# featureform/embeddinghub

Measured on NVIDIA H100. Metric: k-NN queries/s, higher is better.
Workload: dtype f32

## Files before the change

embeddinghub_b200/csrc/api.cu:

```cuda
#include "index_impl.h"

namespace ehb {
thread_local std::string g_err;
int fail(int code, const std::string& msg) {
  g_err = msg;
  return code;
}
const std::string& last_error_text() { return g_err; }
}
using ehb::fail;

ehb_index::~ehb_index() {
  slots.clear();
  if (bf_ev0) cudaEventDestroy(bf_ev0);
  if (bf_ev1) cudaEventDestroy(bf_ev1);
  if (stream) cudaStreamDestroy(stream);
}

ehb::GraphView ehb_index::view() const {
  ehb::GraphView g;
  g.vecs = vecs.p;
  g.links0 = links0.p;
  g.up_off = up_off.p;
  g.links_up = links_up.p;
// ... 24 lines not shown
  const uint64_t need = std::max<uint64_t>(cap, 1) * (dpad + sizeof(float4)) + (256ull << 20);
  bool ok = cudaMemGetInfo(&fr, &tot) == cudaSuccess && fr >= need;
  if (ok) {
    cudaError_t e = x_i8.grow(std::max<uint64_t>(cap, 1) * dpad, 0, -1, stream);
    if (e == cudaSuccess) e = x_i8t.grow(std::max<uint64_t>(cap, 1), 0, -1, stream);
    if (e == cudaSuccess) e = ehb::launch_to_i8(vecs.p, dpad, x_i8.p, x_i8t.p, n, stream);
    if (e == cudaSuccess) e = cudaStreamSynchronize(stream);
    screen_copy = e == cudaSuccess;
    if (!screen_copy) {
      x_i8.release();
      x_i8t.release();
      ok = false;
    }
  }
  if (!ok) {
    (void)cudaGetLastError();
    ehb::g_err.clear();
    screen_no_room = true;
  }
  return EHB_OK;
}

ehb::WalkCfg ehb_index::walk_cfg(uint32_t ef_eff, uint32_t smem_list, uint64_t jobs, uint32_t team, bool bf16,
                                 bool dense) const {
  ehb::WalkCfg c;
  const uint32_t vbytes = dpad * (bf16 ? 2u : 4u);
  c.lcap = smem_list;
  c.staged = ehb::row_lpv(vbytes) == 32 ? 1 : 0;
  c.dcap = n_deleted ? ehb::kDeletedQueue : 0;
  c.prefetch = o_walk_prefetch ? 1 : 0;
  c.dense = dense ? 1 : 0;
  const uint32_t warp_target = c.dense ? 20u : 16u;
  uint32_t nslots = std::max(4u, std::min(32u, 24576u / vbytes));
  uint32_t ng = 2;
  uint32_t g = std::max(4u, nslots / ng / 4 * 4);
  if (t_slots) g = std::min(32u, t_slots);
  if (t_groups) ng = std::min(8u, t_groups);
  c.G = std::max(1u, g);
  c.NG = std::max(1u, ng);
  const uint32_t roomy = 2u * M0 * ef_eff + 64u, tight = std::max(256u, M0 * ef_eff / 4u);
  uint32_t hs = roomy;
  if (t_hash_bits) {
    hs = 1u << t_hash_bits;
  } else {
    uint64_t ctas = (jobs + team - 1) / std::max(team, 1u);
    uint32_t want = (uint32_t)std::min<uint64_t>((ctas + sms - 1) / sms, c.staged ? 5u : warp_target / team);
    want = std::max(want, 4u);
    c.hash_size = 0;
    uint32_t fixed = ehb::warp_smem_bytes(c, vbytes) * team + 1024u + (smem_list ? 256u : 0u);
    uint32_t per_cta = (227u * 1024u) / want;
    uint32_t avail = per_cta > fixed + 1024u ? (per_cta - fixed) / 4u : 256u;
    hs = std::min(roomy, std::max(tight, avail));
    if (n_deleted) hs = roomy;
  }
  c.hash_size = ehb::align_up(std::max(hs, 256u), 32);
  while (ehb::warp_smem_bytes(c, vbytes) + 256 > 200 * 1024 && c.hash_size > 512)
    c.hash_size = ehb::align_up(c.hash_size / 2, 32);
  return c;
}

uint32_t ehb_index::wpb_for(const ehb::WalkCfg& c, uint32_t extra, bool bf16) const {
  uint32_t w = t_wpb ? t_wpb : 1;
  const uint32_t vbytes = dpad * (bf16 ? 2u : 4u);
  while (w > 1 && (size_t)(ehb::warp_smem_bytes(c, vbytes) + extra) * w > 220 * 1024) w >>= 1;
  return w;
}

constexpr uint64_t kTeamWideMaxQueries = 132u * 3u;

ehb::WalkPlan ehb_index::walk_plan(uint64_t nq, uint32_t ef_eff, bool bf16) const {
  ehb::WalkPlan p;
  p.bf16 = bf16;
  const uint32_t row_bytes = dpad * (bf16 ? 2u : 4u);
  p.lpv = ehb::row_lpv(row_bytes);
  p.nq = ehb::row_nq(dpad, row_bytes);
  p.kpl = ehb::kpl_for(ef_eff);
  p.hasdel = n_deleted != 0;
  uint32_t team = t_team;
  if (team == 0) team = nq <= (uint64_t)sms * 3 ? 4 : (nq <= (uint64_t)sms * 7 ? 2 : 1);
  if (dpad > 256 || ef_eff > 256 || n_deleted) team = 1;
  if (bf16) team = 1;
  p.T = team;
  const bool wide = team == 2 || (team == 4 && nq <= kTeamWideMaxQueries);
  p.U = team == 1 ? 0 : (uint32_t)ehb::eval_u(p.nq, wide ? 1 : 2);
  if (team > 1)
    p.form = ehb::WalkForm::team;
  else if (nq >= 20ull * (uint64_t)sms && ehb::dense_form(bf16, p.lpv, p.nq, p.kpl, p.hasdel))
    p.form = ehb::WalkForm::dense;
  else
    p.form = ehb::WalkForm::plain;
  p.screen = !bf16 && team == 1 && screen_copy && walk_screens(nq);
  p.cfg = walk_cfg(ef_eff, 0, nq * team, team, bf16, p.form == ehb::WalkForm::dense);
  p.wpb = wpb_for(p.cfg, 0, bf16);
  return p;
}

int ehb_index::ensure_capacity(uint64_t want) {
  if (want <= cap) return EHB_OK;
  uint64_t nc = std::max<uint64_t>(cap ? cap : 1, 1);
  while (nc < want) nc *= 2;
  if (nc >= 0x7FFFFFFFull) return fail(EHB_ERR_INVALID, "capacity must stay below 2^31 vectors per index");
  CU(vecs.grow(nc * dpad, n * dpad, -1, stream));
  CU(labels.grow(nc, n, -1, stream));
  CU(levels.grow(nc, n, 0, stream));
  CU(deleted.grow(nc, n, 0, stream));
  CU(links0.grow(nc * M0, n * M0, 0xFF, stream));
  CU(up_off.grow(nc, n, 0xFF, stream));
  if (shadow) {
    CU(x_bf16.grow(nc * dpad, n * dpad, -1, stream));
    CU(x_norm.grow(nc, n, -1, stream));
  }
  if (screen_copy) {
    CU(x_i8.grow(nc * dpad, n * dpad, -1, stream));
    CU(x_i8t.grow(nc, n, -1, stream));
  }
// ... 1128 lines not shown
```

embeddinghub_b200/csrc/index_impl.h:

```cpp
#pragma once
#include <cuda_runtime.h>

#include <algorithm>
#include <atomic>
#include <cmath>
#include <condition_variable>
#include <cstdio>
#include <cstdlib>
#include <cstring>
#include <deque>
#include <memory>
#include <mutex>
#include <new>
#include <random>
#include <shared_mutex>
#include <string>
#include <unordered_map>
#include <vector>

#include "../../include/ehb200.h"
#include "kernels.h"

namespace ehb {

// ... 214 lines not shown
  bool shadow = false;
  ehb::DevBuf<int8_t> x_i8;
  ehb::DevBuf<float4> x_i8t;
  bool screen_copy = false;

  ehb::DevBuf<uint32_t> b_edge_row, b_edge_src, b_row_cnt, b_row_fill, b_row_start, b_touched, b_seg_src, b_counters,
      b_ids, b_upd_cand;
  ehb::DevBuf<float> b_edge_dist, b_seg_dist, b_stage_in;

  uint32_t t_slots = 0, t_groups = 0, t_hash_bits = 0, t_wpb = 0, t_team = 0;
  uint32_t o_build_frac = 0;
  bool o_bf16_unfused = false;
  bool o_combine = true;
  bool o_walk_prefetch = false;
  int o_walk_screen = -1;
  bool screen_no_room = false;

  std::default_random_engine level_rng;

  ~ehb_index();

  ehb::GraphView view() const;
  ehb::WalkCfg walk_cfg(uint32_t ef_eff, uint32_t smem_list, uint64_t jobs, uint32_t team, bool bf16 = false,
                        bool dense = false) const;
  uint32_t wpb_for(const ehb::WalkCfg& c, uint32_t extra, bool bf16 = false) const;
  ehb::WalkPlan walk_plan(uint64_t nq, uint32_t ef_eff, bool bf16) const;
  int ensure_capacity(uint64_t want);
  int ensure_upper(uint64_t want_rows);
  int draw_level();
  bool find_id(uint64_t label, uint32_t* id) const;
  int add_rows(uint64_t cnt, const float* src, bool src_is_device, const uint64_t* lab);
  int remove_labels(uint64_t cnt, const uint64_t* lab);
  int ensure_build_scratch(uint64_t edges, uint32_t batch, bool updates);
  ehb::BuildBuffers build_buffers(uint64_t edges);
  ehb::BuildGraph build_graph() const;
  int build();
  int compact();
  bool needs_build() const { return n_linked != n || !pending_updates.empty(); }
  int ensure_built(std::shared_lock<ehb::RwLock>& lk, bool bf16 = false, bool screen = false);
  bool walk_screens(uint64_t nq) const;
  int try_screen_copy();
  int ensure_shadow(std::shared_lock<ehb::RwLock>& lk);
  int create_shadow();
  int derive_rows(uint64_t first, uint64_t cnt);
  void drop_derived();
  int acquire_slot(ehb::SearchSlot** out);
  void release_slot(ehb::SearchSlot* sl, cudaStream_t used);
// ... 8 lines not shown
```

embeddinghub_b200/csrc/search_impl.cuh:

```cuda
#pragma once
#include "kernels.h"

namespace ehb {

template <int LPV, int NQ, int KPL, bool HASDEL, int UDIV, class RowT>
__device__ __forceinline__ void search_body(const GraphView& g, const WalkCfg& cfg, const float* __restrict__ queries,
                                            uint32_t nq, uint32_t k, uint32_t ef, const ResultSink& sink,
                                            uint32_t* __restrict__ out_counts, uint32_t* __restrict__ stats,
                                            uint32_t warp_smem) {
  extern __shared__ __align__(128) unsigned char smem[];
  const uint32_t w = threadIdx.x >> 5;
  const uint32_t q = blockIdx.x * (blockDim.x >> 5) + w;
  if (q >= nq) return;
  constexpr bool kKeys = !std::is_same<RowT, float>::value;
  WarpCtx c;
  ctx_init(c, smem + (size_t)w * warp_smem, cfg, g.dpad, (uint32_t)sizeof(RowT));
  float4 qr[NQ];
  load_query_regs<LPV, NQ, RowT>(qr, queries + (size_t)q * g.dim, g.dim, c.lane);
  WalkCounters wc = {0, 0, 0, 0};
  UList<KPL> ul;
  ul_clear<KPL>(ul, ef, c.lane);
  if (g.n != 0) {
    uint32_t cur = g.entry;
    if (c.lane == 0) c.cand_id[0] = cur;
    __syncwarp();
    eval_candidates<LPV, NQ, UDIV>(c, walk_rows<RowT>(g), qr, 1, g.metric);
    float curdist = c.cand_dist[0];
    __syncwarp();
    wc.evals = 1;
    greedy_descent<LPV, NQ, UDIV, RowT>(c, g, qr, cur, curdist, g.max_level, 0, wc);
    beam_search<LPV, NQ, KPL, true, HASDEL, UDIV, RowT>(c, g, qr, ul, cur, curdist, 0, ef, kInvalid, wc);
  }
  uint64_t rk[KPL];
#pragma unroll
  for (int s = 0; s < KPL; ++s) rk[s] = kMaxKey;
  uint32_t found = 0;
  for (uint32_t i = 0; i < k; ++i) {
    uint64_t key = ul_extract_min<KPL>(ul, c.lane);
    if (key == kMaxKey) break;
#pragma unroll
    for (int s = 0; s < KPL; ++s)
      if ((i >> 5) == (uint32_t)s && (i & 31u) == c.lane) rk[s] = key;
    found++;
  }
  if constexpr (kKeys) {
#pragma unroll
    for (int s = 0; s < KPL; ++s) {
      const uint32_t idx = (uint32_t)s * 32u + c.lane;
      if ((uint32_t)s * 32u < k && idx < k) sink.keys[(size_t)q * k + idx] = rk[s];
    }
  } else {
#pragma unroll
    for (int s = 0; s < KPL; ++s) {
      const uint32_t idx = (uint32_t)s * 32u + c.lane;
// ... 11 lines not shown
    if (sink.qs) {
      __threadfence_system();
      __syncwarp();
      if (c.lane == 0) {
        const uint32_t slice = q / sink.qs;
        const uint32_t size = min(sink.qs, nq - slice * sink.qs);
        if (atomicAdd(&sink.slice_count[slice], 1u) + 1u == size) {
          sink.slice_count[slice] = 0;
          __threadfence_system();
          for (uint32_t t = 1; t < sink.n; ++t) st_release_sys(sink.flags[t] + slice, sink.epoch);
        }
      }
    }
  }
  if (c.lane == 0) {
    if (out_counts) out_counts[q] = found;
    if (stats) {
      ((uint4*)stats)[2 * q] = make_uint4(wc.hops_upper, wc.hops_base, wc.evals, wc.overflow);
      ((uint4*)stats)[2 * q + 1] = make_uint4(wc.screened, wc.survivors, 0u, 0u);
    }
  }
}

template <class RowT, int LPV, int NQ>
constexpr int kWalkMinBlocks = std::is_same<RowT, float>::value && !screen_shape(LPV, NQ) ? 0 : 1;
template <int LPV, int NQ, int KPL, bool HASDEL, class RowT>
__global__ void __launch_bounds__(128, (kWalkMinBlocks<RowT, LPV, NQ>))
    hnsw_search_kernel(GraphView g, WalkCfg cfg, const float* __restrict__ queries, uint32_t nq, uint32_t k, uint32_t ef,
                       const __grid_constant__ ResultSink sink, uint32_t* __restrict__ out_counts,
                       uint32_t* __restrict__ stats, uint32_t warp_smem) {
  search_body<LPV, NQ, KPL, HASDEL, 1, RowT>(g, cfg, queries, nq, k, ef, sink, out_counts, stats, warp_smem);
}

template <int LPV, int NQ, int KPL, class RowT>
__global__ void __launch_bounds__(128, 5) hnsw_search_dense_kernel(GraphView g, WalkCfg cfg,
                                                                   const float* __restrict__ queries, uint32_t nq,
                                                                   uint32_t k, uint32_t ef,
                                                                   const __grid_constant__ ResultSink sink,
                                                                   uint32_t* __restrict__ out_counts,
                                                                   uint32_t* __restrict__ stats, uint32_t warp_smem) {
  search_body<LPV, NQ, KPL, false, 2, RowT>(g, cfg, queries, nq, k, ef, sink, out_counts, stats, warp_smem);
}

template <int LPV, int NQ, int KPL, class RowT>
cudaError_t launch_search_t(const WalkPlan& p, const GraphView& g, const float* queries, uint32_t nq, uint32_t k,
                            uint32_t ef, const ResultSink& sink, uint32_t* out_counts, uint32_t* stats,
                            cudaStream_t s) {
  constexpr bool kBf16 = !std::is_same<RowT, float>::value;
  const uint32_t wpb = p.wpb;
  uint32_t wsm = warp_smem_bytes(p.cfg, g.dpad * (uint32_t)sizeof(RowT));
  size_t smem = (size_t)wsm * wpb;
  dim3 grid((nq + wpb - 1) / wpb), block(32 * wpb);
  void (*kern)(GraphView, WalkCfg, const float*, uint32_t, uint32_t, uint32_t, const ResultSink, uint32_t*, uint32_t*,
               uint32_t) = p.hasdel ? hnsw_search_kernel<LPV, NQ, KPL, true, RowT>
                                    : hnsw_search_kernel<LPV, NQ, KPL, false, RowT>;
  if (p.form == WalkForm::dense) {
    if (!dense_form(kBf16, LPV, NQ, KPL, p.hasdel)) return cudaErrorInvalidValue;
    if constexpr (dense_form(kBf16, LPV, NQ, KPL, false)) kern = hnsw_search_dense_kernel<LPV, NQ, KPL, RowT>;
  }
  cudaError_t e = cudaFuncSetAttribute(kern, cudaFuncAttributeMaxDynamicSharedMemorySize, (int)smem);
  if (e != cudaSuccess) return e;
  kern<<<grid, block, smem, s>>>(g, p.cfg, queries, nq, k, ef, sink, out_counts, stats, wsm);
  return cudaGetLastError();
}

template <uint32_t DPAD, class RowT>
cudaError_t SearchShape<DPAD, RowT>::launch(const WalkPlan& p, const GraphView& g, const float* queries, uint32_t nq,
                                            uint32_t k, uint32_t ef, const ResultSink& sink, uint32_t* out_counts,
                                            uint32_t* stats, cudaStream_t s) {
  constexpr int LPV = row_lpv(DPAD * sizeof(RowT)), NQ = row_nq(DPAD, DPAD * sizeof(RowT));
  if (p.lpv != LPV || p.nq != NQ || p.form == WalkForm::team) return cudaErrorInvalidValue;
  switch (p.kpl) {
    case 2: return launch_search_t<LPV, NQ, 2, RowT>(p, g, queries, nq, k, ef, sink, out_counts, stats, s);
    case 4: return launch_search_t<LPV, NQ, 4, RowT>(p, g, queries, nq, k, ef, sink, out_counts, stats, s);
    case 8: return launch_search_t<LPV, NQ, 8, RowT>(p, g, queries, nq, k, ef, sink, out_counts, stats, s);
    case 16: return launch_search_t<LPV, NQ, 16, RowT>(p, g, queries, nq, k, ef, sink, out_counts, stats, s);
    default: return cudaErrorInvalidValue;
  }
}

}
```

embeddinghub_b200/csrc/walk.cuh:

```cuda
#pragma once
#include <cuda_bf16.h>

#include <type_traits>

#include "common.cuh"

namespace ehb {

struct GraphView {
  const float* vecs;
  const uint32_t* links0;
  const uint32_t* up_off;
  const uint32_t* links_up;
  const uint64_t* labels;
  const uint8_t* deleted;
  uint32_t n, dim, dpad, M, M0, entry;
  int32_t max_level;
  int32_t metric;
  const __nv_bfloat16* vecs16;
  const int8_t* codes8;
  const float4* terms8;
};

struct WalkCfg {
// ... 46 lines not shown

__host__ __device__ inline uint32_t warp_smem_bytes(const WalkCfg& c, uint32_t vbytes) {
  uint32_t b = 0;
  b += align_up(c.lcap * 8u, 128);
  b += align_up(c.hash_size * 4u, 128);
  b += 128;
  b += 128;
  b += 128;
  b += align_up(c.dcap * 8u, 128);
  b += c.staged ? align_up(c.G * c.NG * vbytes, 128) : 0u;
  return b;
}

struct WarpCtx {
  uint64_t* keys;
  uint32_t* hash;
  uint32_t* cand_id;
  float* cand_dist;
  uint64_t* mbar;
  uint32_t* dq_hi;
  uint32_t* dq_id;
  float* stage;
  uint32_t lcap, hsize, G, NG, dpad, vbytes, dcap, prefetch;
  uint32_t phases;
  uint32_t cnt;
  uint32_t lane;
};

__device__ __forceinline__ void ctx_init(WarpCtx& c, unsigned char* base, const WalkCfg& cfg, uint32_t dpad,
                                         uint32_t esize = 4u) {
  c.lane = lane_id();
  c.lcap = cfg.lcap;
  c.G = cfg.G;
  c.NG = cfg.NG;
  c.dpad = dpad;
  c.vbytes = dpad * esize;
  c.hsize = cfg.hash_size;
  unsigned char* p = base;
  c.keys = (uint64_t*)p;
  p += align_up(cfg.lcap * 8u, 128);
  c.hash = (uint32_t*)p;
  p += align_up(cfg.hash_size * 4u, 128);
  c.cand_id = (uint32_t*)p;
  p += 128;
  c.cand_dist = (float*)p;
  p += 128;
  c.mbar = (uint64_t*)p;
  p += 128;
  c.dcap = cfg.dcap;
  c.prefetch = cfg.prefetch;
  c.dq_hi = (uint32_t*)p;
  c.dq_id = c.dq_hi + cfg.dcap;
  p += align_up(cfg.dcap * 8u, 128);
  c.stage = (float*)p;
  c.phases = 0;
  c.cnt = 0;
  if (cfg.staged) {
    if (c.lane < cfg.NG) mbar_init(&c.mbar[c.lane], 1);
    fence_mbar_init();
  }
  __syncwarp();
}

__device__ __forceinline__ void hash_clear(WarpCtx& c) {
  uint4* h4 = (uint4*)c.hash;
  uint32_t n4 = c.hsize >> 2;
  for (uint32_t i = c.lane; i < n4; i += 32) h4[i] = make_uint4(kInvalid, kInvalid, kInvalid, kInvalid);
  __syncwarp();
}

__device__ __forceinline__ bool hash_insert(WarpCtx& c, uint32_t id, uint32_t& overflow) {
  uint32_t h = __umulhi(id * 0x9E3779B1u, c.hsize);
#pragma unroll 1
  for (int probe = 0; probe < 8; ++probe) {
    uint32_t old = atomicCAS(&c.hash[h], kInvalid, id);
    if (old == kInvalid) return true;
    if (old == id) return false;
    h = h + 1u == c.hsize ? 0u : h + 1u;
  }
  overflow = 1;
  return true;
}

template <class RowT, int NQ, int W = (std::is_same<RowT, __nv_bfloat16>::value && NQ > 1) ? 8 : 4>
struct LaneChunks {
  static_assert(W == 4 || (W == 8 && std::is_same<RowT, __nv_bfloat16>::value), "no such chunk");
  using T = std::conditional_t<std::is_same<RowT, float>::value, float4,
                               std::conditional_t<std::is_same<RowT, int8_t>::value, uint32_t,
                                                  std::conditional_t<W == 8, uint4, uint2>>>;
  static constexpr int V = W / 4;
  static constexpr int N = NQ / V;
};
__device__ __forceinline__ float4 ld_chunk(const float4* p) { return ld_nc_f4(p); }
__device__ __forceinline__ uint4 ld_chunk(const uint4* p) { return ld_nc_u4(p); }
__device__ __forceinline__ uint2 ld_chunk(const uint2* p) { return ld_nc_u2(p); }
__device__ __forceinline__ float4 bf16x4_to_f4(uint32_t a, uint32_t b) {
  return make_float4(__uint_as_float(a << 16), __uint_as_float(a & 0xFFFF0000u), __uint_as_float(b << 16),
                     __uint_as_float(b & 0xFFFF0000u));
}
__device__ __forceinline__ void widen(const float4& v, float4* x) { x[0] = v; }
__device__ __forceinline__ void widen(const uint4& v, float4* x) {
  x[0] = bf16x4_to_f4(v.x, v.y);
  x[1] = bf16x4_to_f4(v.z, v.w);
}
__device__ __forceinline__ void widen(const uint2& v, float4* x) { x[0] = bf16x4_to_f4(v.x, v.y); }
__device__ __forceinline__ void widen(const uint32_t& v, float4* x) {
  const uint32_t u = v ^ 0x80808080u;
  x[0] = make_float4(__uint_as_float(__byte_perm(u, 0x4B000000u, 0x7540)) - 8388736.0f,
                     __uint_as_float(__byte_perm(u, 0x4B000000u, 0x7541)) - 8388736.0f,
                     __uint_as_float(__byte_perm(u, 0x4B000000u, 0x7542)) - 8388736.0f,
                     __uint_as_float(__byte_perm(u, 0x4B000000u, 0x7543)) - 8388736.0f);
}

template <int LPV, int NQ, class RowT = float>
__device__ __forceinline__ void load_query_regs(float4 (&qr)[NQ], const float* __restrict__ src, uint32_t dim,
                                                uint32_t lane) {
  constexpr int V = LaneChunks<RowT, NQ>::V;
  uint32_t sub = lane % LPV;
#pragma unroll
  for (int t = 0; t < NQ; ++t) {
    uint32_t e = (sub + LPV * (t / V)) * 4u * V + 4u * (t % V);
    float4 v;
    v.x = e + 0 < dim ? src[e + 0] : 0.f;
    v.y = e + 1 < dim ? src[e + 1] : 0.f;
    v.z = e + 2 < dim ? src[e + 2] : 0.f;
    v.w = e + 3 < dim ? src[e + 3] : 0.f;
    qr[t] = v;
  }
}
template <int LPV, int NQ, class RowT, class C = LaneChunks<RowT, NQ>>
__device__ __forceinline__ void load_vec_regs(typename C::T (&r)[C::N], const RowT* __restrict__ row,
                                              uint32_t lane) {
  const typename C::T* p = (const typename C::T*)row + (lane % LPV);
#pragma unroll
  for (int t = 0; t < C::N; ++t) r[t] = p[LPV * t];
// ... 116 lines not shown
        typename LaneChunks<RowT, NQ>::T x[LaneChunks<RowT, NQ>::N];
        load_vec_regs<32, NQ>(x, (const RowT*)c.stage + (size_t)(buf * c.G + v) * c.dpad, c.lane);
        acc[i] = chunk_dist<NQ, RowT>(x, qr, metric);
      }
#pragma unroll
      for (int o = 16; o > 0; o >>= 1) {
#pragma unroll
        for (int i = 0; i < 4; ++i) acc[i] += __shfl_xor_sync(0xffffffffu, acc[i], o);
      }
      if (c.lane < 4 && v0 + c.lane < cnt) {
        float a = c.lane == 0 ? acc[0] : (c.lane == 1 ? acc[1] : (c.lane == 2 ? acc[2] : acc[3]));
        c.cand_dist[first + v0 + c.lane] = metric == 0 ? a : 1.0f - a;
      }
    }
    __syncwarp();
    if (r + c.NG < rounds) {
      fence_proxy_async();
      issue_group(c, vecs, r + c.NG, m);
    }
  }
  __syncwarp();
}

template <int LPV, int NQ, int UDIV = 1, class RowT = float>
__device__ __forceinline__ void eval_candidates(WarpCtx& c, const RowT* __restrict__ vecs, const float4 (&qr)[NQ],
                                                uint32_t m, int metric) {
  if (LPV == 8)
    eval_direct<NQ, eval_u(LaneChunks<RowT, NQ>::N, UDIV)>(c, vecs, qr, m, metric);
  else
    eval_staged<NQ>(c, vecs, qr, m, metric);
}

struct ScreenQuery {
  float l1, l2, a;
};
__device__ __forceinline__ ScreenQuery* screen_query(const WarpCtx& c) { return (ScreenQuery*)(c.mbar + 8); }
template <int NQ>
__device__ __forceinline__ uint32_t screen_staged(WarpCtx& c, const GraphView& g, const float4 (&qr)[NQ], uint32_t m,
                                                  uint32_t worst_hi, uint32_t& unsure) {
  using C = LaneChunks<int8_t, NQ>;
  constexpr int SV = 4;
  const uint32_t G = min(4u * c.G, 32u), vbytes = c.dpad;
  const uint32_t rounds = (m + G - 1) / G;
  const uint32_t pre = min(rounds, c.NG);
  const bool in = c.lane < m;
  fence_proxy_async();
  for (uint32_t r = 0; r < pre; ++r) issue_rows(c, g.codes8, r, m, G, vbytes);
  const uint32_t id = in ? c.cand_id[c.lane] : kInvalid;
  float4 tm = make_float4(0.f, 0.f, 0.f, 0.f);
  if (in) tm = ld_nc_f4(g.terms8 + id);
#pragma unroll 1
  for (uint32_t r = 0; r < rounds; ++r) {
    uint32_t buf = r % c.NG;
    mbar_wait(&c.mbar[buf], (c.phases >> buf) & 1u);
    c.phases ^= (1u << buf);
    uint32_t first = r * G;
    uint32_t cnt = min(G, m - first);
#pragma unroll 1
    for (uint32_t v0 = 0; v0 < cnt; v0 += SV) {
      float e[SV];
#pragma unroll
      for (int i = 0; i < SV; ++i) {
        uint32_t v = min(v0 + (uint32_t)i, cnt - 1u);
        const typename C::T* s4 = (const typename C::T*)((const int8_t*)c.stage + (size_t)(buf * G + v) * c.dpad) +
                                  c.lane;
        float4 x[NQ];
#pragma unroll
        for (int t = 0; t < C::N; ++t) widen(s4[32 * t], x + t);
        e[i] = partial_dist<NQ>(x, qr, 1);
      }
#pragma unroll
      for (int o = 16; o > 0; o >>= 1) {
#pragma unroll
        for (int i = 0; i < SV; ++i) e[i] += __shfl_xor_sync(0xffffffffu, e[i], o);
      }
      if (c.lane < (uint32_t)SV && v0 + c.lane < cnt) {
        float ea = e[0];
#pragma unroll
        for (int i = 1; i < SV; ++i)
          if (c.lane == (uint32_t)i) ea = e[i];
        c.cand_dist[first + v0 + c.lane] = ea;
      }
    }
    __syncwarp();
    if (r + c.NG < rounds) {
      fence_proxy_async();
      issue_rows(c, g.codes8, r + c.NG, m, G, vbytes);
    }
  }
  __syncwarp();
  float L = 0.f;
  if (in) {
    const ScreenQuery sq = *screen_query(c);
    const float e = (float)c.dpad * 0x1p-24f;
    const float gam = __fdiv_ru(e, 1.0f - e), as = __fmul_ru((float)c.dpad, 0x1p-118f);
    const float se = __fmul_ru(tm.x, c.cand_dist[c.lane]);
    float mg = __fmul_ru(__fmul_ru(gam, sq.l2), __fmaf_ru(2.0f, tm.w, tm.z));
    mg = __fadd_ru(mg, fminf(__fmul_ru(sq.l1, tm.y), __fmul_ru(sq.l2, tm.z)));
    mg = __fadd_ru(mg, __fmaf_ru(tm.x, as, sq.a));
    L = __fsub_rd(__fsub_rd(1.0f, se), mg);
  }
  const bool keep = in && !(isfinite(L) && f2ord(L) >= worst_hi);
  const uint32_t mask = __ballot_sync(0xffffffffu, keep);
  const uint32_t pos = __popc(mask & lanemask_lt());
  __syncwarp();
  if (keep) c.cand_id[pos] = id;
  if (unsure) unsure = __reduce_or_sync(0xffffffffu, (keep && ((unsure >> c.lane) & 1u)) ? (1u << pos) : 0u);
  fence_proxy_async();
  __syncwarp();
  return __popc(mask);
}

template <int NQ>
__device__ __forceinline__ void eval_survivors(WarpCtx& c, const float* __restrict__ vecs, const float4 (&qr)[NQ],
                                               uint32_t m) {
  constexpr int SB = NQ <= 24 ? 24 / NQ : 1;
#pragma unroll 1
  for (uint32_t v0 = 0; v0 < m; v0 += SB) {
    float4 x[SB][NQ];
#pragma unroll
    for (int i = 0; i < SB; ++i) {
      const uint32_t v = min(v0 + (uint32_t)i, m - 1u);
      const float4* p = (const float4*)(vecs + (size_t)c.cand_id[v] * c.dpad) + c.lane;
#pragma unroll
      for (int t = 0; t < NQ; ++t) x[i][t] = ld_nc_f4(p + 32 * t);
    }
    float acc[SB];
#pragma unroll
    for (int i = 0; i < SB; ++i) acc[i] = chunk_dist<NQ, float>(x[i], qr, 1);
#pragma unroll
    for (int o = 16; o > 0; o >>= 1) {
#pragma unroll
      for (int i = 0; i < SB; ++i) acc[i] += __shfl_xor_sync(0xffffffffu, acc[i], o);
    }
    if (c.lane < (uint32_t)SB && v0 + c.lane < m) {
      float a = acc[0];
#pragma unroll
      for (int i = 1; i < SB; ++i)
        if (c.lane == (uint32_t)i) a = acc[i];
      c.cand_dist[v0 + c.lane] = 1.0f - a;
    }
  }
  __syncwarp();
}

template <int KPL>
struct UList {
  uint32_t hi[KPL];
  uint32_t id[KPL];
};
template <int KPL>
__device__ __forceinline__ void ul_clear(UList<KPL>& u, uint32_t ef, uint32_t lane) {
#pragma unroll
  for (int s = 0; s < KPL; ++s) {
    u.hi[s] = ((uint32_t)s * 32u + lane) < ef ? 0xFFFFFFFFu : 0u;
    u.id[s] = kInvalid;
  }
}
template <int KPL>
__device__ __forceinline__ uint32_t ul_worst(const UList<KPL>& u) {
  uint32_t m = u.hi[0];
#pragma unroll
  for (int s = 1; s < KPL; ++s) m = max(m, u.hi[s]);
  return __reduce_max_sync(0xffffffffu, m);
}
template <int KPL>
// ... 124 lines not shown
  __syncwarp();
  c.cnt = newcnt;
  return pos;
}

struct WalkCounters {
  uint32_t hops_upper, hops_base, evals, overflow, screened, survivors;
};

__device__ __forceinline__ uint32_t load_row(const GraphView& g, uint32_t node, int level, uint32_t lane) {
  const uint32_t* row;
  uint32_t width;
  if (level == 0) {
    row = g.links0 + (size_t)node * g.M0;
    width = g.M0;
  } else {
    row = g.links_up + (size_t)(g.up_off[node] + (uint32_t)(level - 1)) * g.M;
    width = g.M;
  }
  uint32_t v = row[min(lane, width - 1u)];
  return lane < width ? v : kInvalid;
}

template <int LPV, int NQ, int UDIV = 1, class RowT = float>
__device__ __forceinline__ void greedy_descent(WarpCtx& c, const GraphView& g, const float4 (&qr)[NQ], uint32_t& cur,
                                               float& curdist, int from_level, int to_level_excl,
                                               WalkCounters& wc) {
  for (int level = from_level; level > to_level_excl; --level) {
    bool changed = true;
    while (changed) {
      changed = false;
      __syncwarp();
      uint32_t nb = load_row(g, cur, level, c.lane);
      uint32_t mask = __ballot_sync(0xffffffffu, nb != kInvalid);
      uint32_t m = __popc(mask);
      wc.hops_upper++;
      if (!m) break;
      if (nb != kInvalid) c.cand_id[__popc(mask & lanemask_lt())] = nb;
      __syncwarp();
      wc.evals += m;
      eval_candidates<LPV, NQ, UDIV>(c, walk_rows<RowT>(g), qr, m, g.metric);
      float bd = c.lane < m ? c.cand_dist[c.lane] : INFINITY;
      uint32_t bl = c.lane;
#pragma unroll
      for (int o = 16; o > 0; o >>= 1) {
        float od = __shfl_xor_sync(0xffffffffu, bd, o);
        uint32_t ol = __shfl_xor_sync(0xffffffffu, bl, o);
        if (od < bd || (od == bd && ol < bl)) bd = od, bl = ol;
      }
      if (bd < curdist) {
        curdist = bd;
        cur = c.cand_id[bl];
        changed = true;
      }
      __syncwarp();
    }
  }
}

__device__ __forceinline__ void dq_push(WarpCtx& c, uint32_t& dn, uint32_t hi, uint32_t id, uint32_t bound,
                                        uint32_t& overflow) {
  if (dn < c.dcap) {
    if (c.lane == 0) c.dq_hi[dn] = hi, c.dq_id[dn] = id;
    dn++;
  } else {
    uint32_t w = 0, wp = 0;
    for (uint32_t i = c.lane; i < dn; i += 32)
      if (c.dq_hi[i] >= w) w = c.dq_hi[i], wp = i;
    uint32_t wm = __reduce_max_sync(0xffffffffu, w);
    uint32_t b = __ballot_sync(0xffffffffu, w == wm);
    uint32_t pos = __shfl_sync(0xffffffffu, wp, __ffs(b) - 1);
    if (hi < wm && c.lane == 0) c.dq_hi[pos] = hi, c.dq_id[pos] = id;
    if (max(hi, wm) <= bound) overflow = 1;
  }
  __syncwarp();
}
__device__ __forceinline__ uint32_t dq_min(const WarpCtx& c, uint32_t dn, uint32_t& hi_out) {
  uint32_t m = 0xFFFFFFFFu, mp = kInvalid;
  for (uint32_t i = c.lane; i < dn; i += 32)
    if (c.dq_hi[i] < m) m = c.dq_hi[i], mp = i;
  uint32_t mm = __reduce_min_sync(0xffffffffu, m);
  uint32_t b = __ballot_sync(0xffffffffu, m == mm && mp != kInvalid);
  hi_out = mm;
  return b ? __shfl_sync(0xffffffffu, mp, __ffs(b) - 1) : kInvalid;
}

template <int LPV, int NQ, int KPL, bool PREFETCH, bool HASDEL, int UDIV = 1, class RowT = float>
__device__ __forceinline__ void beam_search(WarpCtx& c, const GraphView& g, const float4 (&qr)[NQ], UList<KPL>& u,
                                            uint32_t ep, float epdist, int level, uint32_t ef, uint32_t exclude,
                                            WalkCounters& wc) {
  constexpr bool kScreen = screen_shape(LPV, NQ) && std::is_same<RowT, float>::value;
  const bool screen = kScreen && g.codes8 && g.metric == 1;
  if (screen) {
    float mx = 0.f, l1 = 0.f, l2 = 0.f;
#pragma unroll
    for (int t = 0; t < NQ; ++t) {
      const float v[4] = {qr[t].x, qr[t].y, qr[t].z, qr[t].w};
#pragma unroll
      for (int j = 0; j < 4; ++j) {
        mx = fmaxf(mx, fabsf(v[j]));
        l1 = __fadd_ru(l1, fabsf(v[j]));
        l2 = __fmaf_ru(v[j], v[j], l2);
      }
    }
#pragma unroll
    for (int o = 16; o > 0; o >>= 1) {
      l1 = __fadd_ru(l1, __shfl_xor_sync(0xffffffffu, l1, o));
      l2 = __fadd_ru(l2, __shfl_xor_sync(0xffffffffu, l2, o));
    }
    mx = __uint_as_float(__reduce_max_sync(0xffffffffu, __float_as_uint(mx)));
    if (c.lane == 0)
      *screen_query(c) = {l1, __fsqrt_ru(l2), __fmul_ru((float)g.dpad, __fmaf_ru(mx, 0x1p-125f, 0x1p-124f))};
    __syncwarp();
  }
  hash_clear(c);
  ul_clear<KPL>(u, ef, c.lane);
  const uint8_t* __restrict__ del = (HASDEL && c.dcap) ? g.deleted : nullptr;
  uint32_t dn = 0;
  uint32_t ovf = 0;
  if (c.lane == 0) {
    hash_insert(c, ep, ovf);
    if (exclude != kInvalid) hash_insert(c, exclude, ovf);
  }
  __syncwarp();
  uint32_t cnt = 0;
  uint32_t worst_hi = 0xFFFFFFFFu;
  bool ovf_any = false;
  const bool ep_result = ep != exclude && !(del && del[ep]);
  if (ep_result) ul_insert<KPL>(u, f2ord(epdist), ep, ef, cnt, worst_hi, c.lane);
  uint32_t node = ep;
  if (ep_result) node = ul_min_unexpanded<KPL>(u, true, c.lane);
  uint32_t nb = load_row(g, node, level, c.lane);
  for (;;) {
    if (level == 0) wc.hops_base++; else wc.hops_upper++;
    if (HASDEL && wc.hops_base + wc.hops_upper > 64u * ef + 65536u) break;
    __syncwarp();
    const uint32_t spec = ul_min_unexpanded<KPL>(u, false, c.lane);
    uint32_t spec_row = kInvalid;
    if (spec != kInvalid) spec_row = load_row(g, spec & kIdMask, level, c.lane);
    bool is_new = false;
    uint32_t o = 0;
    if (nb != kInvalid && nb != exclude) is_new = hash_insert(c, nb, o);
    ovf |= o;
    __syncwarp();
    uint32_t mask = __ballot_sync(0xffffffffu, is_new);
    uint32_t m = __popc(mask);
    if (m) {
      const uint32_t pos = __popc(mask & lanemask_lt());
      if (is_new) c.cand_id[pos] = nb;
      uint32_t unsure = (HASDEL && del) ? __reduce_or_sync(0xffffffffu, (is_new && o) ? (1u << pos) : 0u) : 0u;
      __syncwarp();
      wc.evals += m;
      if (kScreen && screen && cnt >= ef) {
        wc.screened += m;
        m = screen_staged<NQ>(c, g, qr, m, worst_hi, unsure);
        wc.survivors += m;
        eval_survivors<NQ>(c, g.vecs, qr, m);
      } else {
        eval_candidates<LPV, NQ, UDIV>(c, walk_rows<RowT>(g), qr, m, g.metric);
      }
      if (PREFETCH && LPV == 8 && c.prefetch && spec_row != kInvalid) {
        const char* pv = (const char*)(walk_rows<RowT>(g) + (size_t)spec_row * g.dpad);
#pragma unroll
        for (int b = 0; b < NQ * 8 * 16 * (int)sizeof(RowT) / 4; b += 128) prefetch_l2(pv + b);
      }
      uint32_t myhi = 0xFFFFFFFFu, myid = kInvalid;
      if (c.lane < m) myhi = f2ord(c.cand_dist[c.lane]), myid = c.cand_id[c.lane];
      const bool mydel = HASDEL && del && c.lane < m && del[myid];
      __syncwarp();
      ovf_any = ovf_any || __any_sync(0xffffffffu, ovf);
      uint32_t qual = __ballot_sync(0xffffffffu, c.lane < m && (cnt < ef || myhi < worst_hi));
      const uint32_t delmask = (HASDEL && del) ? __ballot_sync(0xffffffffu, mydel) : 0u;
      while (qual) {
        int j = __ffs(qual) - 1;
        qual &= qual - 1;
        uint32_t hj = __shfl_sync(0xffffffffu, myhi, j);
        uint32_t ij = __shfl_sync(0xffffffffu, myid, j);
        if (cnt >= ef && hj >= worst_hi) continue;
        if (HASDEL && ((delmask >> j) & 1u)) {
          if (!((unsure >> j) & 1u)) dq_push(c, dn, hj, ij, cnt >= ef ? worst_hi : 0xFFFFFFFFu, ovf);
          continue;
        }
// ... 28 lines not shown
```

Before: 458,900.

## Screen candidates from registers using integer dp4a query quantization

Replaces the TMA/mbarrier-staged int8 screening path with direct register loads of codes and a dp4a dot product against a query quantized into hi/lo int8 parts, with the bound updated to account for query quantization error. Adds a dedicated screen kernel with a register cap, and disables shared-memory staging for screened walks so full-precision evaluation also loads directly into registers. This aims to remove async-copy pipeline and shared-memory staging overhead and to make the int8 screen cheaper. The risks are register pressure and spilling under the cap, less latency hiding without the staged pipeline, and a changed error bound that must stay conservative.

```diff
diff --git a/embeddinghub_b200/csrc/api.cu b/embeddinghub_b200/csrc/api.cu
--- a/embeddinghub_b200/csrc/api.cu
+++ b/embeddinghub_b200/csrc/api.cu
@@ -70,7 +70,7 @@
 }
 
 ehb::WalkCfg ehb_index::walk_cfg(uint32_t ef_eff, uint32_t smem_list, uint64_t jobs, uint32_t team, bool bf16,
-                                 bool dense) const {
+                                 bool dense, bool screen) const {
   ehb::WalkCfg c;
   const uint32_t vbytes = dpad * (bf16 ? 2u : 4u);
   c.lcap = smem_list;
@@ -104,6 +104,7 @@
   c.hash_size = ehb::align_up(std::max(hs, 256u), 32);
   while (ehb::warp_smem_bytes(c, vbytes) + 256 > 200 * 1024 && c.hash_size > 512)
     c.hash_size = ehb::align_up(c.hash_size / 2, 32);
+  if (screen) c.staged = 0;
   return c;
 }
 
@@ -138,7 +139,7 @@
   else
     p.form = ehb::WalkForm::plain;
   p.screen = !bf16 && team == 1 && screen_copy && walk_screens(nq);
-  p.cfg = walk_cfg(ef_eff, 0, nq * team, team, bf16, p.form == ehb::WalkForm::dense);
+  p.cfg = walk_cfg(ef_eff, 0, nq * team, team, bf16, p.form == ehb::WalkForm::dense, p.screen);
   p.wpb = wpb_for(p.cfg, 0, bf16);
   return p;
 }
diff --git a/embeddinghub_b200/csrc/index_impl.h b/embeddinghub_b200/csrc/index_impl.h
--- a/embeddinghub_b200/csrc/index_impl.h
+++ b/embeddinghub_b200/csrc/index_impl.h
@@ -260,7 +260,7 @@
 
   ehb::GraphView view() const;
   ehb::WalkCfg walk_cfg(uint32_t ef_eff, uint32_t smem_list, uint64_t jobs, uint32_t team, bool bf16 = false,
-                        bool dense = false) const;
+                        bool dense = false, bool screen = false) const;
   uint32_t wpb_for(const ehb::WalkCfg& c, uint32_t extra, bool bf16 = false) const;
   ehb::WalkPlan walk_plan(uint64_t nq, uint32_t ef_eff, bool bf16) const;
   int ensure_capacity(uint64_t want);
diff --git a/embeddinghub_b200/csrc/search_impl.cuh b/embeddinghub_b200/csrc/search_impl.cuh
--- a/embeddinghub_b200/csrc/search_impl.cuh
+++ b/embeddinghub_b200/csrc/search_impl.cuh
@@ -13,6 +13,7 @@
   const uint32_t q = blockIdx.x * (blockDim.x >> 5) + w;
   if (q >= nq) return;
   constexpr bool kKeys = !std::is_same<RowT, float>::value;
+  constexpr bool kScreen = !kKeys && screen_shape(LPV, NQ);
   WarpCtx c;
   ctx_init(c, smem + (size_t)w * warp_smem, cfg, g.dpad, (uint32_t)sizeof(RowT));
   float4 qr[NQ];
@@ -24,12 +25,12 @@
     uint32_t cur = g.entry;
     if (c.lane == 0) c.cand_id[0] = cur;
     __syncwarp();
-    eval_candidates<LPV, NQ, UDIV>(c, walk_rows<RowT>(g), qr, 1, g.metric);
+    eval_candidates<LPV, NQ, UDIV, RowT, kScreen>(c, walk_rows<RowT>(g), qr, 1, g.metric);
     float curdist = c.cand_dist[0];
     __syncwarp();
     wc.evals = 1;
-    greedy_descent<LPV, NQ, UDIV, RowT>(c, g, qr, cur, curdist, g.max_level, 0, wc);
-    beam_search<LPV, NQ, KPL, true, HASDEL, UDIV, RowT>(c, g, qr, ul, cur, curdist, 0, ef, kInvalid, wc);
+    greedy_descent<LPV, NQ, UDIV, RowT, kScreen>(c, g, qr, cur, curdist, g.max_level, 0, wc);
+    beam_search<LPV, NQ, KPL, true, HASDEL, UDIV, RowT, kScreen>(c, g, qr, ul, cur, curdist, 0, ef, kInvalid, wc);
   }
   uint64_t rk[KPL];
 #pragma unroll
@@ -87,14 +88,24 @@
   }
 }
 
-template <class RowT, int LPV, int NQ>
-constexpr int kWalkMinBlocks = std::is_same<RowT, float>::value && !screen_shape(LPV, NQ) ? 0 : 1;
+template <class RowT>
+constexpr int kWalkMinBlocks = std::is_same<RowT, float>::value ? 0 : 1;
 template <int LPV, int NQ, int KPL, bool HASDEL, class RowT>
-__global__ void __launch_bounds__(128, (kWalkMinBlocks<RowT, LPV, NQ>))
+__global__ void __launch_bounds__(128, (kWalkMinBlocks<RowT>))
     hnsw_search_kernel(GraphView g, WalkCfg cfg, const float* __restrict__ queries, uint32_t nq, uint32_t k, uint32_t ef,
                        const __grid_constant__ ResultSink sink, uint32_t* __restrict__ out_counts,
                        uint32_t* __restrict__ stats, uint32_t warp_smem) {
   search_body<LPV, NQ, KPL, HASDEL, 1, RowT>(g, cfg, queries, nq, k, ef, sink, out_counts, stats, warp_smem);
+}
+
+template <int NQ, int KPL>
+constexpr int kScreenWalkRegs = NQ <= 6 && KPL <= 8 ? 200 : 255;
+template <int LPV, int NQ, int KPL, bool HASDEL>
+__global__ void __maxnreg__((kScreenWalkRegs<NQ, KPL>))
+    hnsw_search_screen_kernel(GraphView g, WalkCfg cfg, const float* __restrict__ queries, uint32_t nq, uint32_t k,
+                              uint32_t ef, const __grid_constant__ ResultSink sink, uint32_t* __restrict__ out_counts,
+                              uint32_t* __restrict__ stats, uint32_t warp_smem) {
+  search_body<LPV, NQ, KPL, HASDEL, 1, float>(g, cfg, queries, nq, k, ef, sink, out_counts, stats, warp_smem);
 }
 
 template <int LPV, int NQ, int KPL, class RowT>
@@ -107,22 +118,32 @@
   search_body<LPV, NQ, KPL, false, 2, RowT>(g, cfg, queries, nq, k, ef, sink, out_counts, stats, warp_smem);
 }
 
+using WalkKernel = void (*)(GraphView, WalkCfg, const float*, uint32_t, uint32_t, uint32_t, const ResultSink,
+                           uint32_t*, uint32_t*, uint32_t);
+template <int LPV, int NQ, int KPL, class RowT>
+WalkKernel walk_kernel(const WalkPlan& p) {
+  constexpr bool kBf16 = !std::is_same<RowT, float>::value;
+  if (p.form == WalkForm::dense) {
+    if constexpr (dense_form(kBf16, LPV, NQ, KPL, false))
+      if (!p.hasdel) return hnsw_search_dense_kernel<LPV, NQ, KPL, RowT>;
+    return nullptr;
+  }
+  if constexpr (std::is_same<RowT, float>::value && screen_shape(LPV, NQ))
+    return p.hasdel ? hnsw_search_screen_kernel<LPV, NQ, KPL, true> : hnsw_search_screen_kernel<LPV, NQ, KPL, false>;
+  else
+    return p.hasdel ? hnsw_search_kernel<LPV, NQ, KPL, true, RowT> : hnsw_search_kernel<LPV, NQ, KPL, false, RowT>;
+}
+
 template <int LPV, int NQ, int KPL, class RowT>
 cudaError_t launch_search_t(const WalkPlan& p, const GraphView& g, const float* queries, uint32_t nq, uint32_t k,
                             uint32_t ef, const ResultSink& sink, uint32_t* out_counts, uint32_t* stats,
                             cudaStream_t s) {
-  constexpr bool kBf16 = !std::is_same<RowT, float>::value;
   const uint32_t wpb = p.wpb;
   uint32_t wsm = warp_smem_bytes(p.cfg, g.dpad * (uint32_t)sizeof(RowT));
   size_t smem = (size_t)wsm * wpb;
   dim3 grid((nq + wpb - 1) / wpb), block(32 * wpb);
-  void (*kern)(GraphView, WalkCfg, const float*, uint32_t, uint32_t, uint32_t, const ResultSink, uint32_t*, uint32_t*,
-               uint32_t) = p.hasdel ? hnsw_search_kernel<LPV, NQ, KPL, true, RowT>
-                                    : hnsw_search_kernel<LPV, NQ, KPL, false, RowT>;
-  if (p.form == WalkForm::dense) {
-    if (!dense_form(kBf16, LPV, NQ, KPL, p.hasdel)) return cudaErrorInvalidValue;
-    if constexpr (dense_form(kBf16, LPV, NQ, KPL, false)) kern = hnsw_search_dense_kernel<LPV, NQ, KPL, RowT>;
-  }
+  const WalkKernel kern = walk_kernel<LPV, NQ, KPL, RowT>(p);
+  if (!kern) return cudaErrorInvalidValue;
   cudaError_t e = cudaFuncSetAttribute(kern, cudaFuncAttributeMaxDynamicSharedMemorySize, (int)smem);
   if (e != cudaSuccess) return e;
   kern<<<grid, block, smem, s>>>(g, p.cfg, queries, nq, k, ef, sink, out_counts, stats, wsm);
diff --git a/embeddinghub_b200/csrc/walk.cuh b/embeddinghub_b200/csrc/walk.cuh
--- a/embeddinghub_b200/csrc/walk.cuh
+++ b/embeddinghub_b200/csrc/walk.cuh
@@ -92,6 +92,7 @@
   uint32_t* dq_id;
   float* stage;
   uint32_t lcap, hsize, G, NG, dpad, vbytes, dcap, prefetch;
+  uint32_t staged;
   uint32_t phases;
   uint32_t cnt;
   uint32_t lane;
@@ -119,6 +120,7 @@
   p += 128;
   c.dcap = cfg.dcap;
   c.prefetch = cfg.prefetch;
+  c.staged = cfg.staged;
   c.dq_hi = (uint32_t*)p;
   c.dq_id = c.dq_hi + cfg.dcap;
   p += align_up(cfg.dcap * 8u, 128);
@@ -155,9 +157,7 @@
 template <class RowT, int NQ, int W = (std::is_same<RowT, __nv_bfloat16>::value && NQ > 1) ? 8 : 4>
 struct LaneChunks {
   static_assert(W == 4 || (W == 8 && std::is_same<RowT, __nv_bfloat16>::value), "no such chunk");
-  using T = std::conditional_t<std::is_same<RowT, float>::value, float4,
-                               std::conditional_t<std::is_same<RowT, int8_t>::value, uint32_t,
-                                                  std::conditional_t<W == 8, uint4, uint2>>>;
+  using T = std::conditional_t<std::is_same<RowT, float>::value, float4, std::conditional_t<W == 8, uint4, uint2>>;
   static constexpr int V = W / 4;
   static constexpr int N = NQ / V;
 };
@@ -174,13 +174,6 @@
   x[1] = bf16x4_to_f4(v.z, v.w);
 }
 __device__ __forceinline__ void widen(const uint2& v, float4* x) { x[0] = bf16x4_to_f4(v.x, v.y); }
-__device__ __forceinline__ void widen(const uint32_t& v, float4* x) {
-  const uint32_t u = v ^ 0x80808080u;
-  x[0] = make_float4(__uint_as_float(__byte_perm(u, 0x4B000000u, 0x7540)) - 8388736.0f,
-                     __uint_as_float(__byte_perm(u, 0x4B000000u, 0x7541)) - 8388736.0f,
-                     __uint_as_float(__byte_perm(u, 0x4B000000u, 0x7542)) - 8388736.0f,
-                     __uint_as_float(__byte_perm(u, 0x4B000000u, 0x7543)) - 8388736.0f);
-}
 
 template <int LPV, int NQ, class RowT = float>
 __device__ __forceinline__ void load_query_regs(float4 (&qr)[NQ], const float* __restrict__ src, uint32_t dim,
@@ -343,82 +336,101 @@
   __syncwarp();
 }
 
-template <int LPV, int NQ, int UDIV = 1, class RowT = float>
+template <int NQ>
+__device__ __forceinline__ void eval_regs(WarpCtx& c, const float* __restrict__ vecs, const float4 (&qr)[NQ],
+                                          uint32_t m, int metric) {
+  constexpr int SB = NQ <= 24 ? 24 / NQ : 1;
+#pragma unroll 1
+  for (uint32_t v0 = 0; v0 < m; v0 += SB) {
+    float4 x[SB][NQ];
+#pragma unroll
+    for (int i = 0; i < SB; ++i) {
+      const uint32_t v = min(v0 + (uint32_t)i, m - 1u);
+      const float4* p = (const float4*)(vecs + (size_t)c.cand_id[v] * c.dpad) + c.lane;
+#pragma unroll
+      for (int t = 0; t < NQ; ++t) x[i][t] = ld_nc_f4(p + 32 * t);
+    }
+    float acc[SB];
+#pragma unroll
+    for (int i = 0; i < SB; ++i) acc[i] = chunk_dist<NQ, float>(x[i], qr, metric);
+#pragma unroll
+    for (int o = 16; o > 0; o >>= 1) {
+#pragma unroll
+      for (int i = 0; i < SB; ++i) acc[i] += __shfl_xor_sync(0xffffffffu, acc[i], o);
+    }
+    if (c.lane < (uint32_t)SB && v0 + c.lane < m) {
+      float a = acc[0];
+#pragma unroll
+      for (int i = 1; i < SB; ++i)
+        if (c.lane == (uint32_t)i) a = acc[i];
+      c.cand_dist[v0 + c.lane] = metric == 0 ? a : 1.0f - a;
+    }
+  }
+  __syncwarp();
+}
+
+template <int LPV, int NQ, int UDIV = 1, class RowT = float, bool SCREEN = false>
 __device__ __forceinline__ void eval_candidates(WarpCtx& c, const RowT* __restrict__ vecs, const float4 (&qr)[NQ],
                                                 uint32_t m, int metric) {
-  if (LPV == 8)
+  if (LPV == 8) {
     eval_direct<NQ, eval_u(LaneChunks<RowT, NQ>::N, UDIV)>(c, vecs, qr, m, metric);
-  else
+  } else {
+    if constexpr (SCREEN) {
+      if (!c.staged) {
+        eval_regs<NQ>(c, vecs, qr, m, metric);
+        return;
+      }
+    }
     eval_staged<NQ>(c, vecs, qr, m, metric);
-}
-
+  }
+}
+
+constexpr int kQMax = 8191;
 struct ScreenQuery {
-  float l1, l2, a;
+  float l1, l2, a, en, sq;
 };
 __device__ __forceinline__ ScreenQuery* screen_query(const WarpCtx& c) { return (ScreenQuery*)(c.mbar + 8); }
 template <int NQ>
-__device__ __forceinline__ uint32_t screen_staged(WarpCtx& c, const GraphView& g, const float4 (&qr)[NQ], uint32_t m,
-                                                  uint32_t worst_hi, uint32_t& unsure) {
-  using C = LaneChunks<int8_t, NQ>;
-  constexpr int SV = 4;
-  const uint32_t G = min(4u * c.G, 32u), vbytes = c.dpad;
-  const uint32_t rounds = (m + G - 1) / G;
-  const uint32_t pre = min(rounds, c.NG);
+__device__ __forceinline__ uint32_t screen_regs(WarpCtx& c, const GraphView& g, const uint32_t (&qh)[NQ],
+                                                const uint32_t (&ql)[NQ], uint32_t m, uint32_t worst_hi,
+                                                uint32_t& unsure) {
+  constexpr int RB = 96 / NQ;
   const bool in = c.lane < m;
-  fence_proxy_async();
-  for (uint32_t r = 0; r < pre; ++r) issue_rows(c, g.codes8, r, m, G, vbytes);
   const uint32_t id = in ? c.cand_id[c.lane] : kInvalid;
   float4 tm = make_float4(0.f, 0.f, 0.f, 0.f);
   if (in) tm = ld_nc_f4(g.terms8 + id);
+  int K = 0;
 #pragma unroll 1
-  for (uint32_t r = 0; r < rounds; ++r) {
-    uint32_t buf = r % c.NG;
-    mbar_wait(&c.mbar[buf], (c.phases >> buf) & 1u);
-    c.phases ^= (1u << buf);
-    uint32_t first = r * G;
-    uint32_t cnt = min(G, m - first);
-#pragma unroll 1
-    for (uint32_t v0 = 0; v0 < cnt; v0 += SV) {
-      float e[SV];
-#pragma unroll
-      for (int i = 0; i < SV; ++i) {
-        uint32_t v = min(v0 + (uint32_t)i, cnt - 1u);
-        const typename C::T* s4 = (const typename C::T*)((const int8_t*)c.stage + (size_t)(buf * G + v) * c.dpad) +
-                                  c.lane;
-        float4 x[NQ];
-#pragma unroll
-        for (int t = 0; t < C::N; ++t) widen(s4[32 * t], x + t);
-        e[i] = partial_dist<NQ>(x, qr, 1);
-      }
-#pragma unroll
-      for (int o = 16; o > 0; o >>= 1) {
-#pragma unroll
-        for (int i = 0; i < SV; ++i) e[i] += __shfl_xor_sync(0xffffffffu, e[i], o);
-      }
-      if (c.lane < (uint32_t)SV && v0 + c.lane < cnt) {
-        float ea = e[0];
-#pragma unroll
-        for (int i = 1; i < SV; ++i)
-          if (c.lane == (uint32_t)i) ea = e[i];
-        c.cand_dist[first + v0 + c.lane] = ea;
-      }
-    }
-    __syncwarp();
-    if (r + c.NG < rounds) {
-      fence_proxy_async();
-      issue_rows(c, g.codes8, r + c.NG, m, G, vbytes);
-    }
-  }
-  __syncwarp();
+  for (uint32_t v0 = 0; v0 < m; v0 += RB) {
+    uint32_t x[RB][NQ];
+#pragma unroll
+    for (int i = 0; i < RB; ++i) {
+      const uint32_t* p = (const uint32_t*)(g.codes8 + (size_t)c.cand_id[min(v0 + (uint32_t)i, m - 1u)] * c.dpad) +
+                          c.lane;
+#pragma unroll
+      for (int t = 0; t < NQ; ++t) x[i][t] = ld_nc_u32(p + 32 * t);
+    }
+#pragma unroll
+    for (int i = 0; i < RB; ++i) {
+      int h = 0, l = 0;
+#pragma unroll
+      for (int t = 0; t < NQ; ++t) {
+        h = __dp4a((int)x[i][t], (int)qh[t], h);
+        l = __dp4a((int)x[i][t], (int)ql[t], l);
+      }
+      const int kv = __reduce_add_sync(0xffffffffu, 128 * h + l);
+      if (c.lane == v0 + (uint32_t)i) K = kv;
+    }
+  }
   float L = 0.f;
   if (in) {
     const ScreenQuery sq = *screen_query(c);
     const float e = (float)c.dpad * 0x1p-24f;
-    const float gam = __fdiv_ru(e, 1.0f - e), as = __fmul_ru((float)c.dpad, 0x1p-118f);
-    const float se = __fmul_ru(tm.x, c.cand_dist[c.lane]);
-    float mg = __fmul_ru(__fmul_ru(gam, sq.l2), __fmaf_ru(2.0f, tm.w, tm.z));
+    const float gam = __fdiv_ru(e, 1.0f - e);
+    const float se = __fmul_ru(__fmul_ru(tm.x, __int2float_ru(K)), sq.sq);
+    float mg = __fmul_ru(__fmul_ru(gam, sq.l2), tm.w);
     mg = __fadd_ru(mg, fminf(__fmul_ru(sq.l1, tm.y), __fmul_ru(sq.l2, tm.z)));
-    mg = __fadd_ru(mg, __fmaf_ru(tm.x, as, sq.a));
+    mg = __fadd_ru(mg, __fmaf_ru(sq.en, __fadd_ru(tm.w, tm.z), sq.a));
     L = __fsub_rd(__fsub_rd(1.0f, se), mg);
   }
   const bool keep = in && !(isfinite(L) && f2ord(L) >= worst_hi);
@@ -427,42 +439,8 @@
   __syncwarp();
   if (keep) c.cand_id[pos] = id;
   if (unsure) unsure = __reduce_or_sync(0xffffffffu, (keep && ((unsure >> c.lane) & 1u)) ? (1u << pos) : 0u);
-  fence_proxy_async();
   __syncwarp();
   return __popc(mask);
-}
-
-template <int NQ>
-__device__ __forceinline__ void eval_survivors(WarpCtx& c, const float* __restrict__ vecs, const float4 (&qr)[NQ],
-                                               uint32_t m) {
-  constexpr int SB = NQ <= 24 ? 24 / NQ : 1;
-#pragma unroll 1
-  for (uint32_t v0 = 0; v0 < m; v0 += SB) {
-    float4 x[SB][NQ];
-#pragma unroll
-    for (int i = 0; i < SB; ++i) {
-      const uint32_t v = min(v0 + (uint32_t)i, m - 1u);
-      const float4* p = (const float4*)(vecs + (size_t)c.cand_id[v] * c.dpad) + c.lane;
-#pragma unroll
-      for (int t = 0; t < NQ; ++t) x[i][t] = ld_nc_f4(p + 32 * t);
-    }
-    float acc[SB];
-#pragma unroll
-    for (int i = 0; i < SB; ++i) acc[i] = chunk_dist<NQ, float>(x[i], qr, 1);
-#pragma unroll
-    for (int o = 16; o > 0; o >>= 1) {
-#pragma unroll
-      for (int i = 0; i < SB; ++i) acc[i] += __shfl_xor_sync(0xffffffffu, acc[i], o);
-    }
-    if (c.lane < (uint32_t)SB && v0 + c.lane < m) {
-      float a = acc[0];
-#pragma unroll
-      for (int i = 1; i < SB; ++i)
-        if (c.lane == (uint32_t)i) a = acc[i];
-      c.cand_dist[v0 + c.lane] = 1.0f - a;
-    }
-  }
-  __syncwarp();
 }
 
 template <int KPL>
@@ -633,7 +611,7 @@
   return lane < width ? v : kInvalid;
 }
 
-template <int LPV, int NQ, int UDIV = 1, class RowT = float>
+template <int LPV, int NQ, int UDIV = 1, class RowT = float, bool SCREEN = false>
 __device__ __forceinline__ void greedy_descent(WarpCtx& c, const GraphView& g, const float4 (&qr)[NQ], uint32_t& cur,
                                                float& curdist, int from_level, int to_level_excl,
                                                WalkCounters& wc) {
@@ -650,7 +628,7 @@
       if (nb != kInvalid) c.cand_id[__popc(mask & lanemask_lt())] = nb;
       __syncwarp();
       wc.evals += m;
-      eval_candidates<LPV, NQ, UDIV>(c, walk_rows<RowT>(g), qr, m, g.metric);
+      eval_candidates<LPV, NQ, UDIV, RowT, SCREEN>(c, walk_rows<RowT>(g), qr, m, g.metric);
       float bd = c.lane < m ? c.cand_dist[c.lane] : INFINITY;
       uint32_t bl = c.lane;
 #pragma unroll
@@ -696,12 +674,13 @@
   return b ? __shfl_sync(0xffffffffu, mp, __ffs(b) - 1) : kInvalid;
 }
 
-template <int LPV, int NQ, int KPL, bool PREFETCH, bool HASDEL, int UDIV = 1, class RowT = float>
+template <int LPV, int NQ, int KPL, bool PREFETCH, bool HASDEL, int UDIV = 1, class RowT = float, bool SCREEN = false>
 __device__ __forceinline__ void beam_search(WarpCtx& c, const GraphView& g, const float4 (&qr)[NQ], UList<KPL>& u,
                                             uint32_t ep, float epdist, int level, uint32_t ef, uint32_t exclude,
                                             WalkCounters& wc) {
-  constexpr bool kScreen = screen_shape(LPV, NQ) && std::is_same<RowT, float>::value;
-  const bool screen = kScreen && g.codes8 && g.metric == 1;
+  static_assert(!SCREEN || (screen_shape(LPV, NQ) && std::is_same<RowT, float>::value), "no screen for this shape");
+  const bool screen = SCREEN && g.codes8 && g.metric == 1;
+  uint32_t qh[NQ], ql[NQ];
   if (screen) {
     float mx = 0.f, l1 = 0.f, l2 = 0.f;
 #pragma unroll
@@ -720,8 +699,30 @@
       l2 = __fadd_ru(l2, __shfl_xor_sync(0xffffffffu, l2, o));
     }
     mx = __uint_as_float(__reduce_max_sync(0xffffffffu, __float_as_uint(mx)));
+    float sq = mx / (float)kQMax;
+    if (!(sq >= 0x1p-126f && sq <= 0x1.fffffep127f)) sq = 0.f;
+    double e2 = 0.0;
+#pragma unroll
+    for (int t = 0; t < NQ; ++t) {
+      const float v[4] = {qr[t].x, qr[t].y, qr[t].z, qr[t].w};
+      uint32_t h = 0, l = 0;
+#pragma unroll
+      for (int j = 0; j < 4; ++j) {
+        const int k = sq != 0.f ? max(-kQMax, min(kQMax, __float2int_rn(v[j] / sq))) : 0;
+        const double e = (double)v[j] - (double)sq * (double)k;
+        e2 = __fma_ru(e, e, e2);
+        const int kh = (k + 64) >> 7;
+        h |= (uint32_t)(kh & 0xFF) << (8 * j);
+        l |= (uint32_t)((k - 128 * kh) & 0xFF) << (8 * j);
+      }
+      qh[t] = h;
+      ql[t] = l;
+    }
+#pragma unroll
+    for (int o = 16; o > 0; o >>= 1) e2 = __dadd_ru(e2, __shfl_xor_sync(0xffffffffu, e2, o));
     if (c.lane == 0)
-      *screen_query(c) = {l1, __fsqrt_ru(l2), __fmul_ru((float)g.dpad, __fmaf_ru(mx, 0x1p-125f, 0x1p-124f))};
+      *screen_query(c) = {l1, __fsqrt_ru(l2), __fmul_ru((float)g.dpad, __fmaf_ru(mx, 0x1p-125f, 0x1p-124f)),
+                          __double2float_ru(__dsqrt_ru(e2)), sq};
     __syncwarp();
   }
   hash_clear(c);
@@ -762,13 +763,13 @@
       uint32_t unsure = (HASDEL && del) ? __reduce_or_sync(0xffffffffu, (is_new && o) ? (1u << pos) : 0u) : 0u;
       __syncwarp();
       wc.evals += m;
-      if (kScreen && screen && cnt >= ef) {
+      if (SCREEN && screen && cnt >= ef) {
         wc.screened += m;
-        m = screen_staged<NQ>(c, g, qr, m, worst_hi, unsure);
+        m = screen_regs<NQ>(c, g, qh, ql, m, worst_hi, unsure);
         wc.survivors += m;
-        eval_survivors<NQ>(c, g.vecs, qr, m);
+        eval_regs<NQ>(c, g.vecs, qr, m, 1);
       } else {
-        eval_candidates<LPV, NQ, UDIV>(c, walk_rows<RowT>(g), qr, m, g.metric);
+        eval_candidates<LPV, NQ, UDIV, RowT, SCREEN>(c, walk_rows<RowT>(g), qr, m, g.metric);
       }
       if (PREFETCH && LPV == 8 && c.prefetch && spec_row != kInvalid) {
         const char* pv = (const char*)(walk_rows<RowT>(g) + (size_t)spec_row * g.dpad);
```

After: 520,700 (median of 6 runs). +13.5%, better.
